# Project-MONAI/GenerativeModels

Measured on AMD Instinct MI355X. Metric: 3D volumes/sec (DDIM 50-step sample, 1x128^3), higher is better.
Workload: dtype bf16; 1 GPU; C2: 3D DiffusionModelUNet(64,128,256; 2 res blocks; mid-block attention 1 head x 256) DDIM-50 sampling of 1x1x128^3 volumes, 1 volume per GPU per step; inference_steps=50, parallelism=1 independent replicas (batch-sharded, no data-path collective), hip_graph=False, self_launched=False

## Files before the change

generativemodels_amd/csrc/small_ops.hip:

```cpp
#include <cstdlib>
#include "attn_common.h"
#include "conv_common.h"

struct LinearRowsExtra {
  const float* ln_g; const float* ln_b; float ln_eps;
  void* y1; void* y2; long long y12_ld; int split;
  const int* off_dev; long long off_mul;
  const float* kv_ws; int kv_dh;
  const float* mlp_p; int mlp_nj; const void* mlp_x1; const float* mlp_b2; void* mlp_x0;
  const float* pre_scale; const float* pre_shift; long long ss_ld; int rows_per_sample;
  void* vt; int vt_c0; int vt_dh;
  const double* gn_stats[2]; int gn_S[2]; int gn_C[2]; const float* gn_gamma; const float* gn_beta; float gn_eps; int gn_groups; int gn_N;
};

__device__ __forceinline__ float kv_merge_one(const float* __restrict__ ws, int BH, int dh, int bh, int c) {
  constexpr int NS = GM_DECODE_KV_SPLITS;
  const float* o = ws + (long long)bh * NS * dh + c;
  const float* m = ws + (long long)BH * NS * dh + (long long)bh * NS;
  const float* l = m + (long long)BH * NS;
  float ms[NS], ls[NS], os[NS];
#pragma unroll
  for (int s = 0; s < NS; ++s) { ms[s] = m[s]; ls[s] = l[s]; os[s] = o[(long long)s * dh]; }
  float M = -INFINITY;
#pragma unroll
// ... 58 lines not shown
    const float* bsrc = bias ? bias : reinterpret_cast<const float*>(w);
    const T* rsrc = res ? res + (long long)(row_ok ? row : 0) * res_ld : w;
#pragma unroll
    for (int i = 0; i < 4; ++i) {
      const int co = co0 + 4 * q + i;
      bia[i] = bsrc[bias ? (co < cout ? co : cout - 1) : 0];
      rsd[i] = ElemIO<T>::ld(rsrc + (res ? (co < cout ? co : cout - 1) : 0));
    }
  }
  f32x4_t acc = (f32x4_t){0.f, 0.f, 0.f, 0.f};
  constexpr int U = 4;
  for (int c0 = 0; c0 < nchunks; c0 += U) {
    uint4 wf[U], xf[U];
    float asc[U][VECW], ash[U][VECW];
#pragma unroll
    for (int u = 0; u < U; ++u) {
      const int c = c0 + u < nchunks ? c0 + u : nchunks - 1;
      wf[u] = *reinterpret_cast<const uint4*>(wrow + (long long)c * cout_pad * BK);
      const bool ok = row_ok & (c * BK + q * VECW + VECW <= cin);
      const uint4 v = *reinterpret_cast<const uint4*>(ok ? xrow + c * BK : x);
      xf[u] = make_uint4(ok ? v.x : 0u, ok ? v.y : 0u, ok ? v.z : 0u, ok ? v.w : 0u);
      if (ex.pre_scale) {
        const int cb = c * BK + q * VECW + VECW <= cin ? c * BK + q * VECW : 0;
        const long long off = (long long)((row_ok ? row : 0) / ex.rows_per_sample) * ex.ss_ld + cb;
#pragma unroll
        for (int i = 0; i < VECW; i += 4) {
          const float4 a = *reinterpret_cast<const float4*>(ex.pre_scale + off + i), b2 = *reinterpret_cast<const float4*>(ex.pre_shift + off + i);
          asc[u][i] = a.x; asc[u][i + 1] = a.y; asc[u][i + 2] = a.z; asc[u][i + 3] = a.w;
          ash[u][i] = b2.x; ash[u][i + 1] = b2.y; ash[u][i + 2] = b2.z; ash[u][i + 3] = b2.w;
        }
      }
    }
#pragma unroll
    for (int u = 0; u < U; ++u) {
      if (c0 + u >= nchunks) break;
      uint4 b = xf[u];
      if (pre_act || ex.ln_g || ex.pre_scale) {
        float v[VECW];
        Vec16<T>::unpack(b, v);
        if (ex.pre_scale) {
          const bool okc = row_ok & ((c0 + u) * BK + q * VECW + VECW <= cin);
#pragma unroll
          for (int i = 0; i < VECW; ++i) v[i] = okc ? v[i] * asc[u][i] + ash[u][i] : 0.f;
        }
        if (ex.ln_g) {
          const int cbase = (c0 + u) * BK + q * VECW;
          const bool ok = row_ok & (cbase + VECW <= cin);
#pragma unroll
          for (int i = 0; i < VECW; ++i) v[i] = ok ? (v[i] - mean) * rstd * ex.ln_g[cbase + i] + (ex.ln_b ? ex.ln_b[cbase + i] : 0.f) : 0.f;
        }
        if (pre_act) {
          conv_act_vec(v, pre_act, PRECISE);
        }
        b = Vec16<T>::pack(v);
      }
      Mma<T>::run(wf[u], b, acc);
    }
  }
  if (!row_ok) return;
#pragma unroll
  for (int i = 0; i < 4; ++i) {
    const int co = co0 + 4 * q + i;
    if (co < cout) {
      float v = acc[i] + (bias ? bia[i] : 0.f);
      v = conv_post_act(v, post_act);
      if (res) v += rsd[i];
      if (ex.split > 0 && co >= ex.split) {
        T* dst = reinterpret_cast<T*>(co < 2 * ex.split ? ex.y1 : ex.y2) + (ex.off_dev ? (long long)(*ex.off_dev) * ex.off_mul : 0);
        ElemIO<T>::st(dst + (long long)row * ex.y12_ld + (co - (co < 2 * ex.split ? ex.split : 2 * ex.split)), v);
      } else {
        ElemIO<T>::st(y + (long long)row * y_ld + co, v);
        if (ex.vt && co >= ex.vt_c0) {
          const int cch = co - ex.vt_c0, L = ex.rows_per_sample;
          const int smp = row / L, key = row - smp * L;
          const int pos = (key & ~31) + ((key & 15) >> 2) * 8 + ((key >> 4) & 1) * 4 + (key & 3);
          const int heads = (cout - ex.vt_c0) / ex.vt_dh;
          ElemIO<T>::st(reinterpret_cast<T*>(ex.vt) + ((long long)(smp * heads + cch / ex.vt_dh) * ex.vt_dh + cch % ex.vt_dh) * L + pos, v);
        }
      }
    }
  }
}

template <typename T, int NB, bool GN>
__global__ __launch_bounds__(256) void token_gemm_wide_kernel(const T* __restrict__ x, long long x_ld, const T* __restrict__ w, const float* __restrict__ bias,
                                                             const T* __restrict__ res, long long res_ld, T* __restrict__ y, long long y_ld, int rows, int cin,
                                                             int cout, int pre_act, int post_act, LinearRowsExtra ex) {
  constexpr int BK = ConvTraits<T>::BK, VECW = ConvTraits<T>::VECW;
  constexpr bool PRECISE = sizeof(T) == 4;
  const int lane = threadIdx.x & 63, wave = threadIdx.x >> 6;
  const int l15 = lane & 15, q = lane >> 4;
  const int cout_pad = (cout + 15) & ~15;
  const int co0 = blockIdx.x * (16 * NB);
  const int r0 = (blockIdx.y * 4 + wave) * 16;
  extern __shared__ __attribute__((aligned(16))) char gn_smem[];
  if constexpr (GN) {
    float* tab = reinterpret_cast<float*>(gn_smem);
    double* csum = reinterpret_cast<double*>(gn_smem + 2 * (size_t)cin * 4);
    const int n = (blockIdx.y * 64) / ex.rows_per_sample;
    const int cpg = cin / ex.gn_groups;
    for (int c = threadIdx.x; c < cin; c += 256) {
      const double2 v = gn_short_channel_sum(ex.gn_stats[0], ex.gn_S[0], ex.gn_C[0], ex.gn_stats[1], ex.gn_S[1], ex.gn_C[1], ex.gn_N, n, c);
      csum[2 * c] = v.x; csum[2 * c + 1] = v.y;
    }
    __syncthreads();
    for (int c = threadIdx.x; c < cin; c += 256) {
      const int g = c / cpg;
      double a = 0.0, b2 = 0.0;
      for (int j = 0; j < cpg; ++j) { a += csum[2 * (g * cpg + j)]; b2 += csum[2 * (g * cpg + j) + 1]; }
      float sc1, sh1;
      gn_short_scale_shift(a, b2, cpg, (long long)ex.rows_per_sample, ex.gn_eps, ex.gn_gamma ? ex.gn_gamma[c] : 1.f, ex.gn_beta ? ex.gn_beta[c] : 0.f, sc1, sh1);
      tab[c] = sc1;
      tab[cin + c] = sh1;
    }
    __syncthreads();
  }
  if (r0 >= rows) return;
  const int row = r0 + l15;
  const bool row_ok = row < rows;
  const int rowc = row_ok ? row : rows - 1;
  const int nchunks = cin / BK;
  const T* xrow = x + (long long)rowc * x_ld + q * VECW;
  int wblk[NB];
#pragma unroll
  for (int nb = 0; nb < NB; ++nb) wblk[nb] = co0 + 16 * nb < cout_pad ? co0 + 16 * nb : cout_pad - 16;
  const T* wrow = w + (long long)l15 * BK + q * VECW;
  const long long aoff = ex.pre_scale ? (long long)(rowc / ex.rows_per_sample) * ex.ss_ld + q * VECW : 0;
  float bia[NB][4];
  uint2 rsd[NB];
  const bool vec4 = (cout & 3) == 0 && (y_ld & 3) == 0 && (reinterpret_cast<uintptr_t>(y) & (4 * sizeof(T) - 1)) == 0 &&
                    (!res || ((res_ld & 3) == 0 && (reinterpret_cast<uintptr_t>(res) & (4 * sizeof(T) - 1)) == 0));
#pragma unroll
  for (int nb = 0; nb < NB; ++nb) {
#pragma unroll
    for (int i = 0; i < 4; ++i) {
      const int co = wblk[nb] + 4 * q + i;
      bia[nb][i] = bias ? bias[co < cout ? co : cout - 1] : 0.f;
    }
    rsd[nb] = make_uint2(0u, 0u);
    if (sizeof(T) == 2 && res && vec4) {
      const int co = wblk[nb] + 4 * q;
      rsd[nb] = *reinterpret_cast<const uint2*>(res + (long long)rowc * res_ld + (co + 3 < cout ? co : 0));
    }
  }
  f32x4_t acc[NB];
#pragma unroll
  for (int nb = 0; nb < NB; ++nb) acc[nb] = (f32x4_t){0.f, 0.f, 0.f, 0.f};
  constexpr int U = 2;
  for (int c0 = 0; c0 < nchunks; c0 += U) {
    uint4 wf[U][NB], xf[U];
    float asc[U][VECW], ash[U][VECW];
#pragma unroll
    for (int u = 0; u < U; ++u) {
      const int c = c0 + u < nchunks ? c0 + u : nchunks - 1;
      xf[u] = *reinterpret_cast<const uint4*>(xrow + c * BK);
#pragma unroll
      for (int nb = 0; nb < NB; ++nb) wf[u][nb] = *reinterpret_cast<const uint4*>(wrow + ((long long)c * cout_pad + wblk[nb]) * BK);
      if (GN) {
        const float* tab = reinterpret_cast<const float*>(gn_smem) + c * BK + q * VECW;
#pragma unroll
        for (int i = 0; i < VECW; i += 4) {
          const float4 a = *reinterpret_cast<const float4*>(tab + i), b2 = *reinterpret_cast<const float4*>(tab + cin + i);
          asc[u][i] = a.x; asc[u][i + 1] = a.y; asc[u][i + 2] = a.z; asc[u][i + 3] = a.w;
          ash[u][i] = b2.x; ash[u][i + 1] = b2.y; ash[u][i + 2] = b2.z; ash[u][i + 3] = b2.w;
        }
      } else if (ex.pre_scale) {
#pragma unroll
        for (int i = 0; i < VECW; i += 4) {
          const float4 a = *reinterpret_cast<const float4*>(ex.pre_scale + aoff + c * BK + i), b2 = *reinterpret_cast<const float4*>(ex.pre_shift + aoff + c * BK + i);
          asc[u][i] = a.x; asc[u][i + 1] = a.y; asc[u][i + 2] = a.z; asc[u][i + 3] = a.w;
          ash[u][i] = b2.x; ash[u][i + 1] = b2.y; ash[u][i + 2] = b2.z; ash[u][i + 3] = b2.w;
        }
      }
    }
#pragma unroll
    for (int u = 0; u < U; ++u) {
      if (c0 + u >= nchunks) break;
      uint4 b = row_ok ? xf[u] : make_uint4(0u, 0u, 0u, 0u);
      if (pre_act || ex.pre_scale || GN) {
        float v[VECW];
        Vec16<T>::unpack(b, v);
        if (ex.pre_scale || GN) {
#pragma unroll
          for (int i = 0; i < VECW; ++i) v[i] = row_ok ? v[i] * asc[u][i] + ash[u][i] : 0.f;
        }
        if (pre_act) conv_act_vec(v, pre_act, PRECISE);
        b = Vec16<T>::pack(v);
      }
#pragma unroll
      for (int nb = 0; nb < NB; ++nb) Mma<T>::run(wf[u][nb], b, acc[nb]);
    }
  }
  if (!row_ok) return;
#pragma unroll
  for (int nb = 0; nb < NB; ++nb) {
    if (co0 + 16 * nb >= cout_pad) break;
    const int cob = co0 + 16 * nb + 4 * q;
    float o[4];
    float rs[4] = {0.f, 0.f, 0.f, 0.f};
    if (res) {
      if (sizeof(T) == 2 && vec4) {
        rs[0] = __uint_as_float(rsd[nb].x << 16); rs[1] = __uint_as_float(rsd[nb].x & 0xffff0000u);
        rs[2] = __uint_as_float(rsd[nb].y << 16); rs[3] = __uint_as_float(rsd[nb].y & 0xffff0000u);
      } else {
#pragma unroll
        for (int i = 0; i < 4; ++i) rs[i] = cob + i < cout ? ElemIO<T>::ld(res + (long long)row * res_ld + cob + i) : 0.f;
      }
    }
#pragma unroll
    for (int i = 0; i < 4; ++i) {
      float v = acc[nb][i] + (bias ? bia[nb][i] : 0.f);
      v = conv_post_act(v, post_act);
      if (res) v += rs[i];
      o[i] = v;
    }
    if (vec4) {
      if (cob < cout) {
        if (sizeof(T) == 2) *reinterpret_cast<uint2*>(y + (long long)row * y_ld + cob) = make_uint2(pack_bf16x2(o[0], o[1]), pack_bf16x2(o[2], o[3]));
        else *reinterpret_cast<float4*>(y + (long long)row * y_ld + cob) = make_float4(o[0], o[1], o[2], o[3]);
      }
    } else {
#pragma unroll
      for (int i = 0; i < 4; ++i)
        if (cob + i < cout) ElemIO<T>::st(y + (long long)row * y_ld + cob + i, o[i]);
    }
    if (ex.vt && cob + 3 >= ex.vt_c0) {
      const int L = ex.rows_per_sample, smp = row / L, key = row - smp * L;
      const int pos = (key & ~31) + ((key & 15) >> 2) * 8 + ((key >> 4) & 1) * 4 + (key & 3);
      const int heads = (cout - ex.vt_c0) / ex.vt_dh;
#pragma unroll
      for (int i = 0; i < 4; ++i) {
        const int cch = cob + i - ex.vt_c0;
        if (cch >= 0 && cob + i < cout)
          ElemIO<T>::st(reinterpret_cast<T*>(ex.vt) + ((long long)(smp * heads + cch / ex.vt_dh) * ex.vt_dh + cch % ex.vt_dh) * L + pos, o[i]);
      }
    }
  }
}

static int gm_token_gemm_wide_rows = 2048, gm_token_gemm_wide_nb = 0;
extern "C" void gm_token_gemm_set_wide(int min_rows, int nb) {
  gm_token_gemm_wide_rows = min_rows < 0 ? 2048 : min_rows;
  gm_token_gemm_wide_nb = (nb == 2 || nb == 3 || nb == 4) ? nb : 0;
}

#define GM_ROWS_KCH 4

template <typename T, bool SRC_LDS>
__device__ __forceinline__ void stage_rows(const T* __restrict__ x, long long x_ld, T* xs, int rows, int cin, const float* __restrict__ ln_g,
                                           const float* __restrict__ ln_b, float ln_eps, int pre_act) {
  constexpr int VECW = ConvTraits<T>::VECW;
  constexpr bool PRECISE = sizeof(T) == 4;
  const int lane = threadIdx.x & 63, wave = threadIdx.x >> 6;
  const float* gsrc = ln_g ? ln_g : reinterpret_cast<const float*>(x ? (const void*)x : (const void*)xs);
  const float* bsrc = ln_b ? ln_b : gsrc;
  const float bmul = ln_b ? 1.f : 0.f;
  for (int r = wave; r < rows; r += 4) {
    float v[GM_ROWS_KCH][VECW], g[GM_ROWS_KCH][VECW], bb[GM_ROWS_KCH][VECW];
    bool ok[GM_ROWS_KCH];
#pragma unroll
    for (int k = 0; k < GM_ROWS_KCH; ++k) {
      const int ch = (k * 64 + lane) * VECW;
      ok[k] = ch + VECW <= cin;
      const int c = ok[k] ? ch : 0;
      const uint4 raw = SRC_LDS ? *reinterpret_cast<const uint4*>(xs + (long long)r * cin + c) : *reinterpret_cast<const uint4*>(x + (long long)r * x_ld + c);
      Vec16<T>::unpack(raw, v[k]);
      if (ln_g) {
#pragma unroll
        for (int i = 0; i < VECW; i += 4) {
          const float4 tg = *reinterpret_cast<const float4*>(gsrc + c + i), tb = *reinterpret_cast<const float4*>(bsrc + c + i);
          g[k][i] = tg.x; g[k][i + 1] = tg.y; g[k][i + 2] = tg.z; g[k][i + 3] = tg.w;
          bb[k][i] = tb.x; bb[k][i + 1] = tb.y; bb[k][i + 2] = tb.z; bb[k][i + 3] = tb.w;
        }
      }
    }
    if (ln_g) {
      float sum = 0.f;
#pragma unroll
      for (int k = 0; k < GM_ROWS_KCH; ++k)
#pragma unroll
        for (int i = 0; i < VECW; ++i) sum += ok[k] ? v[k][i] : 0.f;
      const float mean = wave_sum(sum) / (float)cin;
      float sq = 0.f;
#pragma unroll
      for (int k = 0; k < GM_ROWS_KCH; ++k)
#pragma unroll
        for (int i = 0; i < VECW; ++i) sq += ok[k] ? (v[k][i] - mean) * (v[k][i] - mean) : 0.f;
      const float rstd = 1.0f / sqrtf(wave_sum(sq) / (float)cin + ln_eps);
#pragma unroll
      for (int k = 0; k < GM_ROWS_KCH; ++k)
#pragma unroll
        for (int i = 0; i < VECW; ++i) v[k][i] = (v[k][i] - mean) * rstd * g[k][i] + bb[k][i] * bmul;
    }
#pragma unroll
    for (int k = 0; k < GM_ROWS_KCH; ++k) {
      if (pre_act) conv_act_vec(v[k], pre_act, PRECISE);
      if (ok[k]) *reinterpret_cast<uint4*>(xs + (long long)r * cin + (k * 64 + lane) * VECW) = Vec16<T>::pack(v[k]);
    }
  }
}

template <typename T, int STAGE, int XF>
__global__ __launch_bounds__(256) void linear_rows_ksplit_kernel(const T* __restrict__ x, long long x_ld, const T* __restrict__ w,
                                                                const float* __restrict__ bias, const T* __restrict__ res, long long res_ld,
                                                                T* __restrict__ y, long long y_ld, int rows, int cin, int cout, int pre_act,
                                                                int post_act, LinearRowsExtra ex) {
  constexpr int BK = ConvTraits<T>::BK, VECW = ConvTraits<T>::VECW;
  constexpr bool STAGED = STAGE != 0 || XF != 0;
  __shared__ float part[3][64][4];
  extern __shared__ __attribute__((aligned(16))) char staged_raw[];
  T* xs = reinterpret_cast<T*>(staged_raw);
  const int lane = threadIdx.x & 63, wave = threadIdx.x >> 6;
  const int l15 = lane & 15, q = lane >> 4;
  const int cout_pad = (cout + 15) & ~15;
  const int co0 = blockIdx.x * 16;
  const int row = l15;
  const bool row_ok = row < rows;
  const int nchunks = (cin + BK - 1) / BK;
  const T* wrow = w + ((long long)(co0 + l15)) * BK + q * VECW;
  constexpr int U = 4;
  uint4 wf[U], xf[U];
// ... 142 lines not shown
    const uint4 v = *reinterpret_cast<const uint4*>(xs + (ok ? (long long)row * C + c * BK + q * VECW : 0));
    return make_uint4(ok ? v.x : 0u, ok ? v.y : 0u, ok ? v.z : 0u, ok ? v.w : 0u);
  };
  f32x4_t acc = (f32x4_t){0.f, 0.f, 0.f, 0.f};
  for (int c0 = 0; c0 < nchunks; c0 += U) {
    if (c0 != 0) {
#pragma unroll
      for (int u = 0; u < U; ++u) wf[u] = *reinterpret_cast<const uint4*>(w1row + (long long)(c0 + u < nchunks ? c0 + u : nchunks - 1) * mpad * BK);
    }
#pragma unroll
    for (int u = 0; u < U; ++u)
      if (c0 + u < nchunks) Mma<T>::run(wf[u], xvec(c0 + u), acc);
  }
#pragma unroll
  for (int i = 0; i < 4; ++i) {
    float v = acc[i] + (b1 ? b1v[i] : 0.f);
    v = conv_post_act(v, act);
    ElemIO<T>::st(&hs[l15][wave * 16 + 4 * q + i], row_ok ? v : 0.f);
  }
  __syncthreads();
  uint4 hf[HC];
#pragma unroll
  for (int c = 0; c < HC; ++c) hf[c] = *reinterpret_cast<const uint4*>(&hs[l15][c * BK + q * VECW]);
  float* Pj = P + (long long)j * rows * C;
#pragma unroll
  for (int g = 0; g < GMAX; ++g) {
    const int grp = wave + 4 * g;
    if (grp < ngroups) {
      f32x4_t a2 = (f32x4_t){0.f, 0.f, 0.f, 0.f};
#pragma unroll
      for (int c = 0; c < HC; ++c) Mma<T>::run(w2f[g][c], hf[c], a2);
      if (row_ok) {
#pragma unroll
        for (int i = 0; i < 4; ++i) {
          const int co = grp * 16 + 4 * q + i;
          if (co < C) Pj[(long long)row * C + co] = a2[i];
        }
      }
    }
  }
}

static bool linear_rows_takes_ksplit(int rows, int cin, int dtype) {
  static const bool ksplit = !(getenv("GM_LINEAR_KSPLIT") && getenv("GM_LINEAR_KSPLIT")[0] == '0');
  const int bk = dtype == GM_F32 ? 16 : 32, vecw = dtype == GM_F32 ? 4 : 8;
  return ksplit && (cin + bk - 1) / bk >= 8 && rows <= 16 && cin <= 64 * vecw * GM_ROWS_KCH && (long long)rows * cin * (dtype == GM_F32 ? 4 : 2) <= 48 * 1024;
}

static int linear_rows_launch(const void* x, long long x_ld, const void* w, const float* bias, const void* res, long long res_ld, void* y,
                              long long y_ld, int rows, int cin, int cout, int pre_act, int post_act, int dtype, const LinearRowsExtra& ex,
                              void* stream) {
  GM_REQUIRE((x || ex.kv_ws || ex.mlp_p) && w && y, "null pointer");
  GM_REQUIRE(rows >= 0 && cin > 0 && cout > 0, "bad geometry");
  if (rows == 0) return 0;
  const int vecw = dtype == GM_F32 ? 4 : 8;
  GM_REQUIRE(cin % vecw == 0 && x_ld % vecw == 0 && (reinterpret_cast<uintptr_t>(x) & 15) == 0, "x rows must be 16-byte vectors");
  GM_REQUIRE(!(ex.kv_ws || ex.mlp_p) || linear_rows_takes_ksplit(rows, cin, dtype), "the partial-merging prologues live in the K-split kernel");
  GM_REQUIRE(ex.split == 0 || (ex.y1 && ex.y2 && cout == 3 * ex.split), "split output needs two extra destinations and cout = 3 * split");
  hipStream_t st = (hipStream_t)stream;
  const int cout_pad = (cout + 15) & ~15;
  if (linear_rows_takes_ksplit(rows, cin, dtype) && !ex.pre_scale) {
    dim3 gk(cout_pad / 16, 1);
    const int stage = ex.kv_ws ? 1 : ex.mlp_p ? 2 : 0;
    const int xf = (ex.ln_g || pre_act) ? 1 : 0;
    const size_t smem = (stage || xf) ? (size_t)rows * cin * (dtype == GM_F32 ? 4 : 2) : 0;
#define GM_KSPLIT_LAUNCH(T, STAGE, XF)                                                                                                         \
  linear_rows_ksplit_kernel<T, STAGE, XF><<<gk, 256, smem, st>>>((const T*)x, x_ld, (const T*)w, bias, (const T*)res, res_ld, (T*)y, y_ld, rows, \
                                                                 cin, cout, pre_act, post_act, ex)
#define GM_KSPLIT_DISPATCH(T)                                                         \
  do {                                                                                \
    if (stage == 0) { if (xf) GM_KSPLIT_LAUNCH(T, 0, 1); else GM_KSPLIT_LAUNCH(T, 0, 0); } \
    else if (stage == 1) { if (xf) GM_KSPLIT_LAUNCH(T, 1, 1); else GM_KSPLIT_LAUNCH(T, 1, 0); } \
    else { if (xf) GM_KSPLIT_LAUNCH(T, 2, 1); else GM_KSPLIT_LAUNCH(T, 2, 0); }       \
  } while (0)
    if (dtype == GM_F32) GM_KSPLIT_DISPATCH(float);
    else if (dtype == GM_BF16) GM_KSPLIT_DISPATCH(bf16_raw);
    else GM_FAIL(-2, "unsupported dtype");
#undef GM_KSPLIT_DISPATCH
#undef GM_KSPLIT_LAUNCH
    GM_LAUNCH_CHECK();
  }
  const int bk = dtype == GM_F32 ? 16 : 32;
  const bool gn = ex.gn_stats[0] != nullptr;
  if ((gn || (gm_token_gemm_wide_rows > 0 && rows >= gm_token_gemm_wide_rows)) && cin % bk == 0 && cout_pad >= 32 && !ex.ln_g && !ex.kv_ws && !ex.mlp_p && ex.split == 0 &&
      !ex.off_dev && (!ex.pre_scale || ex.rows_per_sample > 0) && (dtype == GM_F32 || dtype == GM_BF16)) {
    const int nb = gm_token_gemm_wide_nb ? gm_token_gemm_wide_nb : (rows >= 8192 ? 4 : 2);
    dim3 gw((cout_pad + 16 * nb - 1) / (16 * nb), (rows + 63) / 64);
    const size_t gsm = gn ? (size_t)cin * (2 * 4 + 16) : 0;
#define GM_WIDE_LAUNCH(T, NBV)                                                                                                                                    \
  do {                                                                                                                                                            \
    if (gn) token_gemm_wide_kernel<T, NBV, true><<<gw, 256, gsm, st>>>((const T*)x, x_ld, (const T*)w, bias, (const T*)res, res_ld, (T*)y, y_ld, rows, cin, cout, \
                                                                       pre_act, post_act, ex);                                                                    \
    else token_gemm_wide_kernel<T, NBV, false><<<gw, 256, 0, st>>>((const T*)x, x_ld, (const T*)w, bias, (const T*)res, res_ld, (T*)y, y_ld, rows, cin, cout,     \
                                                                   pre_act, post_act, ex);                                                                        \
  } while (0)
    if (dtype == GM_F32) { if (nb == 2) GM_WIDE_LAUNCH(float, 2); else if (nb == 3) GM_WIDE_LAUNCH(float, 3); else GM_WIDE_LAUNCH(float, 4); }
    else { if (nb == 2) GM_WIDE_LAUNCH(bf16_raw, 2); else if (nb == 3) GM_WIDE_LAUNCH(bf16_raw, 3); else GM_WIDE_LAUNCH(bf16_raw, 4); }
#undef GM_WIDE_LAUNCH
    GM_LAUNCH_CHECK();
  }
  GM_REQUIRE(!gn, "the statistics form of the token GEMM's GroupNorm needs the wide kernel's geometry (cin a multiple of the MFMA K step, cout >= 32)");
  dim3 grid((cout_pad / 16 + 3) / 4, (rows + 15) / 16);
  if (dtype == GM_F32)
    linear_rows_kernel<float><<<grid, 256, 0, st>>>((const float*)x, x_ld, (const float*)w, bias, (const float*)res, res_ld, (float*)y, y_ld,
                                                    rows, cin, cout, pre_act, post_act, ex);
  else if (dtype == GM_BF16)
    linear_rows_kernel<bf16_raw><<<grid, 256, 0, st>>>((const bf16_raw*)x, x_ld, (const bf16_raw*)w, bias, (const bf16_raw*)res, res_ld,
                                                       (bf16_raw*)y, y_ld, rows, cin, cout, pre_act, post_act, ex);
  else
    GM_FAIL(-2, "unsupported dtype");
  GM_LAUNCH_CHECK();
}

extern "C" int gm_linear_rows(const void* x, long long x_ld, const void* w, const float* bias, const void* res, long long res_ld, void* y,
                              long long y_ld, int rows, int cin, int cout, int pre_act, int post_act, int dtype, void* stream) {
  LinearRowsExtra ex = {};
  return linear_rows_launch(x, x_ld, w, bias, res, res_ld, y, y_ld, rows, cin, cout, pre_act, post_act, dtype, ex, stream);
}

extern "C" int gm_linear_rows_affine(const void* x, long long x_ld, const float* pre_scale, const float* pre_shift, long long ss_ld, int rows_per_sample,
                                     const void* w, const float* bias, const void* res, long long res_ld, void* y, long long y_ld, int rows, int cin,
                                     int cout, int pre_act, int post_act, int dtype, void* stream) {
  GM_REQUIRE((pre_scale == nullptr) == (pre_shift == nullptr), "scale and shift come together");
  GM_REQUIRE(!pre_scale || (rows_per_sample > 0 && ss_ld % 4 == 0 && (reinterpret_cast<uintptr_t>(pre_scale) & 15) == 0 &&
                            (reinterpret_cast<uintptr_t>(pre_shift) & 15) == 0), "the affine tables are 16-byte aligned fp32 rows");
  LinearRowsExtra ex = {};
  ex.pre_scale = pre_scale; ex.pre_shift = pre_shift; ex.ss_ld = ss_ld; ex.rows_per_sample = rows_per_sample;
  return linear_rows_launch(x, x_ld, w, bias, res, res_ld, y, y_ld, rows, cin, cout, pre_act, post_act, dtype, ex, stream);
}

extern "C" int gm_linear_rows_affine_vt(const void* x, long long x_ld, const float* pre_scale, const float* pre_shift, long long ss_ld, int rows_per_sample,
                                        const void* w, const float* bias, void* y, long long y_ld, int rows, int cin, int cout, int pre_act, void* vt,
                                        int vt_c0, int vt_dh, int dtype, void* stream) {
  GM_REQUIRE((pre_scale == nullptr) == (pre_shift == nullptr), "scale and shift come together");
  GM_REQUIRE(!pre_scale || (ss_ld % 4 == 0 && (reinterpret_cast<uintptr_t>(pre_scale) & 15) == 0 && (reinterpret_cast<uintptr_t>(pre_shift) & 15) == 0),
             "the affine tables are 16-byte aligned fp32 rows");
  GM_REQUIRE(vt && dtype == GM_BF16 && rows_per_sample > 0 && rows_per_sample % 64 == 0 && rows % rows_per_sample == 0, "the V^T image needs bf16 and whole 64-key blocks per sample");
  GM_REQUIRE(vt_dh > 0 && vt_c0 >= 0 && vt_c0 < cout && (cout - vt_c0) % vt_dh == 0, "the V columns are whole heads");
  LinearRowsExtra ex = {};
  ex.pre_scale = pre_scale; ex.pre_shift = pre_shift; ex.ss_ld = ss_ld; ex.rows_per_sample = rows_per_sample;
  ex.vt = vt; ex.vt_c0 = vt_c0; ex.vt_dh = vt_dh;
  return linear_rows_launch(x, x_ld, w, bias, nullptr, 0, y, y_ld, rows, cin, cout, pre_act, 0, dtype, ex, stream);
}

extern "C" int gm_linear_rows_gn(const void* x, long long x_ld, const GmGnTables* gn, int n_samples, int rows_per_sample, const void* w, const float* bias,
                                 const void* res, long long res_ld, void* y, long long y_ld, int rows, int cin, int cout, int pre_act, int post_act, void* vt,
                                 int vt_c0, int vt_dh, int dtype, void* stream) {
  GM_REQUIRE(gn && gn->stats[0] && gn->groups > 0 && cin % gn->groups == 0 && cin <= 384, "GroupNorm tables: whole groups, at most 384 channels");
  GM_REQUIRE(gn->S[0] >= 1 && gn->S[0] <= GN_SHORT_MAX_ROWS && gn->C[0] > 0 &&
             ((gn->stats[1] == nullptr && gn->C[0] == cin) || (gn->stats[1] != nullptr && gn->S[1] >= 1 && gn->S[1] <= GN_SHORT_MAX_ROWS && gn->C[1] > 0 && gn->C[0] + gn->C[1] == cin)),
             "short statistic tables covering the input channels");
  GM_REQUIRE((reinterpret_cast<uintptr_t>(gn->stats[0]) & 15) == 0 && (reinterpret_cast<uintptr_t>(gn->stats[1]) & 15) == 0, "16-byte aligned tables");
  GM_REQUIRE(n_samples > 0 && rows_per_sample > 0 && rows_per_sample % 64 == 0 && rows == n_samples * rows_per_sample, "whole 64-row groups per sample");
  GM_REQUIRE(!vt || (dtype == GM_BF16 && vt_dh > 0 && vt_c0 >= 0 && vt_c0 < cout && (cout - vt_c0) % vt_dh == 0 && !res && post_act == 0), "the V^T image: bf16, whole heads, no residual");
  LinearRowsExtra ex = {};
  ex.rows_per_sample = rows_per_sample;
  ex.gn_stats[0] = gn->stats[0]; ex.gn_stats[1] = gn->stats[1]; ex.gn_S[0] = gn->S[0]; ex.gn_S[1] = gn->stats[1] ? gn->S[1] : 0;
  ex.gn_C[0] = gn->C[0]; ex.gn_C[1] = gn->stats[1] ? gn->C[1] : 0;
  ex.gn_gamma = gn->gamma; ex.gn_beta = gn->beta; ex.gn_eps = gn->eps; ex.gn_groups = gn->groups; ex.gn_N = n_samples;
  ex.vt = vt; ex.vt_c0 = vt_c0; ex.vt_dh = vt_dh;
  return linear_rows_launch(x, x_ld, w, bias, res, res_ld, y, y_ld, rows, cin, cout, pre_act, post_act, dtype, ex, stream);
}

extern "C" int gm_linear_rows_ln(const void* x, long long x_ld, const float* ln_g, const float* ln_b, float ln_eps, const void* w,
                                 const float* bias, void* y, long long y_ld, void* y1, void* y2, long long y12_ld, int split, int rows, int cin,
                                 int cout, int post_act, int dtype, const int* off_dev, long long off_mul, void* stream) {
// ... 526 lines not shown
```

generativemodels_amd/ops.py:

```python
from __future__ import annotations

import contextlib
import ctypes as C
import math
import os
import threading
import weakref
from typing import Optional, Sequence

import torch

from . import _native as nat
from ._native import GmAttnBwdDesc, GmAttnDesc, GmConvDesc, GmGnTables, GmKlParams, GmStepParams, GmWgradDesc, check, lib

_DT = {torch.float32: 0, torch.bfloat16: 1}
ACT = {"none": 0, "silu": 1, "relu": 2}
ACT_BWD = {"none": 0, "silu": 1, "relu": 2, "leakyrelu": 3}
POST_ACT = {"none": 0, "relu": 1, "tanh": 2, "sigmoid": 3, "silu": 4, "swish": 4, "leakyrelu": 5, "gelu": 6}


def dt_code(dtype: torch.dtype) -> int:
    try:
        return _DT[dtype]
    except KeyError:
# ... 605 lines not shown
    if GN_APPLY_POLICY == "prologue":
        return True
    if GN_APPLY_POLICY == "pass":
        return False
    if x.dtype != torch.bfloat16 or x.shape[-1] % 8 != 0:
        return True
    if x.numel() >= (1 << 22):
        return False
    vox = x.numel() // max(x.shape[0] * x.shape[-1], 1)
    return not (x.dim() == 5 and x.shape[-1] % 32 == 0 and vox <= 4096)


def layernorm(x: torch.Tensor, gamma: Optional[torch.Tensor], beta: Optional[torch.Tensor], eps: float = 1e-5) -> torch.Tensor:
    require_device(x)
    out = torch.empty(x.shape, dtype=x.dtype, device=x.device)
    check(lib().gm_layernorm(x.data_ptr(), arena_ld(x), out.data_ptr(), arena_ld(out), _ptr(as_f32(gamma)), _ptr(as_f32(beta)),
                             rows_of(x), x.shape[-1], float(eps), dt_code(x.dtype), _stream()), "gm_layernorm")
    return out


def geglu(x: torch.Tensor) -> torch.Tensor:
    require_device(x)
    inner = x.shape[-1] // 2
    out = torch.empty((*x.shape[:-1], inner), dtype=x.dtype, device=x.device)
    check(lib().gm_geglu(x.data_ptr(), arena_ld(x), out.data_ptr(), arena_ld(out), rows_of(x), inner, dt_code(x.dtype), _stream()),
          "gm_geglu")
    return out


def _clog2(v: int) -> int:
    return max(0, (int(v) - 1).bit_length())


def _tile_bits(total_bits: int, out_dims):
    caps = [_clog2(d) for d in out_dims]
    bits = [0, 0, 0]
    for _ in range(total_bits):
        cand = [i for i in (2, 1, 0) if bits[i] < caps[i]]
        if not cand:
            bits[2] += 1
            continue
        i = min(cand, key=lambda j: bits[j])
        bits[i] += 1
    return bits


def _tile_bits_fast(total_bits: int, out_dims):
    caps = [_clog2(d) for d in out_dims]
    bits = [0, 0, min(4, caps[2], total_bits)]
    for _ in range(total_bits - bits[2]):
        cand = [i for i in (1, 0) if bits[i] < caps[i]]
        if not cand:
            bits[2] += 1
            continue
        i = min(cand, key=lambda j: bits[j])
        bits[i] += 1
    return bits


_CFG_TILES = {}


def _cfg_tile(cfg: int):
    if cfg not in _CFG_TILES:
        bm, bn = C.c_int(), C.c_int()
        check(lib().gm_conv_cfg_tile(cfg, C.byref(bm), C.byref(bn)), "gm_conv_cfg_tile")
        _CFG_TILES[cfg] = (bm.value, bn.value)
    return _CFG_TILES[cfg]


COUT1_MARCH_LTD = os.environ.get("GM_CONV_COUT1_LTD")
COUT1_MARCH_LTW_128B = int(os.environ.get("GM_CONV_COUT1_LTW", "4"))


_CONV_DEBUG_FLAGS = 0
_SK_STAMPS = None
_CONV_TIMELINE_BUFFER = None

SMALL_LINEAR_ROWS = 64
TOKEN_GEMM = os.environ.get("GM_TOKEN_GEMM", "1") != "0"
TOKEN_GEMM_MAX_ROWS = int(os.environ.get("GM_TOKEN_GEMM_MAX_ROWS", "32768"))
TOKEN_GEMM_MAX_CIN = 512
TOKEN_GEMM_MAX_FLOP = float(os.environ.get("GM_TOKEN_GEMM_MAX_FLOP", "2.0e9"))
DMA_CONV = True
DMA_CONV_MIN_VOXELS = 1 << 8
LDS_SOFT_LIMIT = 80 * 1024
LDS_HARD_LIMIT = 160 * 1024


def _choose_conv_cfg(desc: GmConvDesc, n_vox_out: int, force_cfg: Optional[int] = None, only: Optional[tuple] = None, exclude: tuple = ()):
    cout = desc.Cout
    if force_cfg is not None:
        order = [force_cfg]
    elif cout <= 16:
        order = [3, 4, 2]
    elif cout <= 64:
        order = [10, 8, 5, 0, 4, 2] if n_vox_out * desc.N >= (1 << 20) else [8, 5, 0, 4, 2]
    else:
        order = [10, 9, 6, 1, 4, 2] if n_vox_out * desc.N >= (1 << 20) else [9, 6, 1, 4, 2]
    if force_cfg is None and n_vox_out * desc.N >= DMA_CONV_MIN_VOXELS:
        if cout == 1:
            order = ([20, 13] if COUT1_MARCH else [13]) + order
        if desc.Cin <= 4:
            order = [12] + order
    if force_cfg is None and cout > 16 and DMA_CONV and n_vox_out * desc.N >= DMA_CONV_MIN_VOXELS:
        tiles = desc.N * -(-desc.Do // 4) * -(-desc.Ho // 4) * -(-desc.Wo // 16) * -(-cout // 64)
        wide = (bool(desc.pre_scale is None or not desc.pre_scale) or DMA_WIDE_WAVES_PRE) and tiles >= DMA_WIDE_WAVE_MIN_TILES and DMA_WIDE_WAVES
        order = ([15] if desc.sd == 2 else ([14, 11] if wide else [11])) + order
    if (force_cfg is None and NARROW_N_2D and DMA_CONV and desc.kd == 1 and desc.Ds == 1 and desc.kh == 3 and desc.kw == 3
            and ((desc.sh == 1 and desc.sw == 1) or (NARROW_N_2D_STRIDE2 and desc.sh == 2 and desc.sw == 2))
            and 2.0 * n_vox_out * desc.N * cout * desc.Cin * 9 * desc.sh * desc.sw <= NARROW_N_2D_MAX_FLOP):
        order = [25] + order
    if force_cfg is None and n_vox_out * desc.N <= 256 * 64:
        dma_first = [c for c in order if c in (11, 12, 15, 18, 19)]
        rest = [c for c in order if c not in (11, 12, 15, 18, 19)]
        order = dma_first + [c for c in rest if _cfg_tile(c)[0] <= 64] + [c for c in rest if _cfg_tile(c)[0] > 64]
    order = [c for c in order if (only is None or c in only) and c not in exclude]
    best = None
    for cfg in order:
        bm, _ = _cfg_tile(cfg)
        tb = _tile_bits_fast if cfg >= 5 else _tile_bits
        bits = tb(bm.bit_length() - 1, (desc.Do, desc.Ho, desc.Wo))
        if cfg == 20:
            ltw = (COUT1_MARCH_LTW_128B if desc.Cin * (4 if desc.dtype == 0 else 2) == 128 else 4)
            cols = desc.N * -(-desc.Ho // 8) * -(-desc.Wo // (1 << ltw))
            want = 512 if (ltw == 4 and desc.Cin * (4 if desc.dtype == 0 else 2) == 128) else 256
            ltd = 5
            while ltd > 2 and cols * -(-desc.Do // (1 << ltd)) < want:
                ltd -= 1
            if COUT1_MARCH_LTD is not None:
                ltd = int(COUT1_MARCH_LTD)
            bits = [ltd, 3, ltw]
        if cfg in (11, 12, 14, 15, 16, 18, 19, 24, 25):
            bits = {11: [2, 2, 4], 12: [2, 2, 4], 14: [2, 2, 4], 15: [1, 2, 4], 16: [3, 2, 4], 18: [3, 2, 4], 19: [3, 2, 4], 24: [2, 2, 4], 25: [0, 4, 4]}[cfg]
        desc.cfg, desc.ltd, desc.lth, desc.ltw = cfg, bits[0], bits[1], bits[2]
        lds = lib().gm_conv_lds_bytes(C.byref(desc))
        soft = LDS_HARD_LIMIT if cfg >= 5 else LDS_SOFT_LIMIT
        if 0 < lds <= soft:
            return
        if 0 < lds <= LDS_HARD_LIMIT and best is None:
            best = (cfg, bits)
    if best is None:
        raise ValueError("convolution geometry needs more than 160 KiB of LDS per tile (kernel/stride/dilation too large)")
    desc.cfg, (desc.ltd, desc.lth, desc.ltw) = best[0], best[1]


def _attach_conv_stats(d: GmConvDesc, out: torch.Tensor, n: int, cout: int) -> None:
    slots = lib().gm_conv_stats_slots(C.byref(d))
    if slots > 0:
        cst = torch.empty((slots, n, cout, 2), dtype=torch.float64, device=out.device)
        d.stats = cst.data_ptr()
        out._gm_cstats = cst


def _conv_subpixel(x, weight, bias, rowvec, res, post_act, out, want_stats, n, cin, cout, src, packed=None, label="mode3 (executed flops: 8 of the 27 taps)"):
    dtype = x.dtype
    out_sp = tuple(2 * v for v in src)
    out_shape = (n, *out_sp, cout)
    if out is None:
        out = torch.empty(out_shape, dtype=dtype, device=x.device)
    elif tuple(out.shape) != out_shape or out.dtype != dtype:
        raise ValueError(f"out has shape {tuple(out.shape)}, expected {out_shape}")
    d = GmConvDesc()
    if packed is None:
        packed = packed_subpixel_weight(weight, dtype)
    d.in_mode, d.fd, d.fh, d.fw = 3, 2, 2, 2
# ... 73 lines not shown
        x, x2 = x.parts
    require_device(x, x2, weight, bias, rowvec, res, out)
    nsp = x.dim() - 2
    if nsp < 1 or nsp > 3:
        raise ValueError("conv expects (N, *spatial, C) with 1-3 spatial axes")

    def two_pass():
        parts = [x] if x2 is None else [x, x2]
        if pre is None and x2 is None:
            raise AssertionError
        xa = torch.empty((*x.shape[:-1], sum(t.shape[-1] for t in parts)), dtype=x.dtype, device=x.device)
        off = 0
        for t in parts:
            c_t = t.shape[-1]
            if pre is not None:
                gn_apply(t, pre[0][:, off:off + c_t], pre[1][:, off:off + c_t], pre_act, out=xa[..., off:off + c_t])
            else:
                copy_channels(t, xa[..., off:off + c_t])
            off += c_t
        return conv(xa, weight, bias, kernel=kernel, stride=stride, padding=padding, dilation=dilation, pad_hi=pad_hi, upsample=upsample,
                    transposed=transposed, output_padding=output_padding, rowvec=rowvec, res=res, post_act=post_act, out=out, packed=packed,
                    cout=cout, force_cfg=force_cfg, want_stats=want_stats, skip=skip, allow_subpixel=allow_subpixel, ksplit=ksplit, vt=vt)

    def tup(v):
        v = tuple(v) if isinstance(v, (tuple, list)) else (int(v),) * nsp
        if len(v) != nsp:
            raise ValueError("per-axis argument has the wrong length")
        return v

    def pad3(v, fill):
        return (fill,) * (3 - nsp) + tuple(v)

    k = pad3(tup(kernel), 1)
    s = pad3(tup(stride), 1)
    plo = pad3(tup(padding), 0)
    phi = pad3(tup(pad_hi if pad_hi is not None else padding), 0)
    dil = pad3(tup(dilation), 1)
    opad = pad3(tup(output_padding), 0)
    n, cin = x.shape[0], x.shape[-1] + (0 if x2 is None else x2.shape[-1])
    src = pad3(tuple(x.shape[1:-1]), 1)
    dtype = x.dtype
    if x2 is not None and (x2.shape[:-1] != x.shape[:-1] or x2.dtype != dtype):
        raise ValueError("the two parts of a concatenated input must agree outside the channel dim")
    if packed is None:
        cout = weight.shape[1] if transposed else weight.shape[0]
        wcin = weight.shape[0] if transposed else weight.shape[1]
        if wcin != cin:
            raise ValueError(f"input has {cin} channels but the weight expects {wcin}")

    def panel():
        return packed if packed is not None else packed_conv_weight(weight, dtype, transposed)
    rows = n * math.prod(src)
    vecw = 16 // x.element_size()
    if (rows <= SMALL_LINEAR_ROWS and x2 is None and k == (1, 1, 1) and s == (1, 1, 1) and not transposed and not upsample and pre is None
            and rowvec is None and not want_stats and skip is None and force_cfg is None and cin % vecw == 0
            and arena_ld(x) % vecw == 0 and x.data_ptr() % 16 == 0 and plo == (0, 0, 0) and phi == (0, 0, 0)):
        out_shape = (*x.shape[:-1], cout)
        if out is None:
            out = torch.empty(out_shape, dtype=dtype, device=x.device)
        elif tuple(out.shape) != out_shape or out.dtype != dtype:
            raise ValueError(f"out has shape {tuple(out.shape)}, expected {out_shape}")
        if res is not None and (tuple(res.shape) != out_shape or res.dtype != dtype):
            raise ValueError(f"residual has shape {tuple(res.shape)} / {res.dtype}, expected {out_shape} / {dtype}")
        b32 = as_f32(bias) if bias is not None else None
        _timed(f"linear_rows<{str(dtype).split('.')[-1]}>", dict(flops=2.0 * rows * cin * cout, bytes=float(x.element_size() * cin * cout), shape=f"{rows}x{cin}->{cout}"),
               lambda: check(lib().gm_linear_rows(x.data_ptr(), arena_ld(x), panel().data_ptr(), _ptr(b32), _ptr(res), 0 if res is None else arena_ld(res),
                                                  out.data_ptr(), arena_ld(out), rows, cin, cout, ACT[pre_act], POST_ACT[post_act], dt_code(dtype),
                                                  _stream()), "gm_linear_rows"))
        return out
    if (EDGE_2D_AS_3D and nsp == 2 and x2 is None and packed is None and weight is not None and weight.dim() == 4 and not transposed and not upsample
            and cin <= 4 and k == (1, 3, 3) and s == (1, 1, 1) and dil == (1, 1, 1) and plo == (0, 1, 1) and phi == (0, 1, 1) and pre is None
            and pre_act == "none" and skip is None and force_cfg is None and ksplit is None and cout % vecw == 0 and rows >= DMA_CONV_MIN_VOXELS):
        def embed():
            w5 = torch.zeros((weight.shape[0], weight.shape[1], 3, 3, 3), dtype=weight.dtype, device=weight.device)
            w5[:, :, 1] = weight.detach()
            return w5
        got = conv(x.unsqueeze(1), _cached(weight, ("centre_plane_3d",), embed), bias, kernel=3, padding=1, rowvec=rowvec,
                   res=None if res is None else res.unsqueeze(1), post_act=post_act, out=None if out is None else out.unsqueeze(1), want_stats=want_stats)
        y = out if out is not None else got.squeeze(1)
        st = getattr(got, "_gm_cstats", None)
        if st is not None:
            y._gm_cstats = st
        return y
    if (TOKEN_GEMM and SMALL_LINEAR_ROWS < rows <= TOKEN_GEMM_MAX_ROWS and cin <= TOKEN_GEMM_MAX_CIN and 2.0 * rows * cin * cout <= TOKEN_GEMM_MAX_FLOP
            and x2 is None and k == (1, 1, 1) and s == (1, 1, 1) and not upsample and rowvec is None and not want_stats and skip is None
            and force_cfg is None and ksplit is None and cin % vecw == 0 and arena_ld(x) % vecw == 0 and x.data_ptr() % 16 == 0
            and plo == (0, 0, 0) and phi == (0, 0, 0) and opad == (0, 0, 0)):
        out_shape = (*x.shape[:-1], cout)
        if out is None:
            out = torch.empty(out_shape, dtype=dtype, device=x.device)
        elif tuple(out.shape) != out_shape or out.dtype != dtype:
            raise ValueError(f"out has shape {tuple(out.shape)}, expected {out_shape}")
        if res is not None and (tuple(res.shape) != out_shape or res.dtype != dtype):
            raise ValueError(f"residual has shape {tuple(res.shape)} / {res.dtype}, expected {out_shape} / {dtype}")
        b32 = as_f32(bias) if bias is not None else None
        if GN_IN_TOKEN_GEMM and isinstance(pre, GnRecipe) and pre._done is None and not transposed:
            l_tok = rows // n
            want_vt = (vt is not None and res is None and post_act == "none" and dtype == torch.bfloat16 and l_tok % 64 == 0)
            if (pre.n == n and sum(pre.cs) == cin and cin <= 384 and cin % (64 // x.element_size()) == 0 and cout >= 32 and l_tok % 64 == 0
                    and cin % pre.groups == 0 and all(st.shape[0] <= GN_IN_CONSUMER_MAX_ROWS for st in pre.stats) and (vt is None or want_vt)):
                g = GmGnTables()
                for i, st in enumerate(pre.stats):
                    g.stats[i], g.S[i], g.C[i] = st.data_ptr(), st.shape[0], pre.cs[i]
                g.gamma, g.beta, g.eps, g.groups = _ptr(pre.gamma), _ptr(pre.beta), pre.eps, pre.groups
                vws, vt_c0, vt_dh = vt if want_vt else (None, 0, 0)
                _timed(f"token_gemm<{str(dtype).split('.')[-1]}>", dict(flops=2.0 * rows * cin * cout, bytes=float(x.element_size() * (rows * (cin + cout) + cin * cout)),
                                                                      shape=f"{rows}x{cin}->{cout} (GroupNorm from statistics{' +V^T image' if want_vt else ''})"),
                       lambda: check(lib().gm_linear_rows_gn(x.data_ptr(), arena_ld(x), C.byref(g), n, l_tok, panel().data_ptr(), _ptr(b32), _ptr(res),
                                                             0 if res is None else arena_ld(res), out.data_ptr(), arena_ld(out), rows, cin, cout, ACT[pre_act],
                                                             POST_ACT[post_act], None if vws is None else vws.data_ptr(), int(vt_c0), int(vt_dh), dt_code(dtype),
                                                             _stream()), "gm_linear_rows_gn"))
                if want_vt:
                    out._gm_vt_packed = True
                return out
        sc = sh = None
        if pre is not None:
            sc, sh = pre
            if sc.dtype != torch.float32 or sh.dtype != torch.float32 or sc.shape != (n, cin) or sh.shape != (n, cin) or sc.stride(-1) != 1 or sh.stride(-1) != 1 \
                    or sc.stride(0) != sh.stride(0):
                raise ValueError("pre = (scale, shift): fp32 [N, Cin] tables with a common row pitch")
        if (vt is not None and res is None and post_act == "none" and dtype == torch.bfloat16 and (rows // n) % 64 == 0
                and (sc is None or (sc.stride(0) % 4 == 0 and sc.data_ptr() % 16 == 0 and sh.data_ptr() % 16 == 0))):
            vws, vt_c0, vt_dh = vt
            _timed(f"token_gemm<{str(dtype).split('.')[-1]}>", dict(flops=2.0 * rows * cin * cout, bytes=float(x.element_size() * (rows * (cin + cout) + cin * cout)),
                                                                  shape=f"{rows}x{cin}->{cout} (+V^T image)"),
                   lambda: check(lib().gm_linear_rows_affine_vt(x.data_ptr(), arena_ld(x), _ptr(sc), _ptr(sh), 0 if sc is None else sc.stride(0), rows // n,
                                                                panel().data_ptr(), _ptr(b32), out.data_ptr(), arena_ld(out), rows, cin, cout, ACT[pre_act],
                                                                vws.data_ptr(), int(vt_c0), int(vt_dh), dt_code(dtype), _stream()), "gm_linear_rows_affine_vt"))
            out._gm_vt_packed = True
            return out
        if sc is None or (sc.stride(0) % 4 == 0 and sc.data_ptr() % 16 == 0 and sh.data_ptr() % 16 == 0):
            _timed(f"token_gemm<{str(dtype).split('.')[-1]}>", dict(flops=2.0 * rows * cin * cout, bytes=float(x.element_size() * (rows * (cin + cout) + cin * cout)),
                                                                  shape=f"{rows}x{cin}->{cout}"),
                   lambda: check(lib().gm_linear_rows_affine(x.data_ptr(), arena_ld(x), _ptr(sc), _ptr(sh), 0 if sc is None else sc.stride(0), rows // n,
                                                             panel().data_ptr(), _ptr(b32), _ptr(res), 0 if res is None else arena_ld(res), out.data_ptr(),
                                                             arena_ld(out), rows, cin, cout, ACT[pre_act], POST_ACT[post_act], dt_code(dtype), _stream()),
                                 "gm_linear_rows_affine"))
            return out
    if (upsample and x2 is None and SUBPIXEL_UPSAMPLE and allow_subpixel and nsp == 3 and k == (3, 3, 3) and s == (1, 1, 1) and plo == (1, 1, 1) and phi == (1, 1, 1)
            and dil == (1, 1, 1) and pre is None and pre_act == "none" and skip is None and force_cfg is None and weight is not None
            and cin % (64 // x.element_size()) == 0 and cout % vecw == 0 and arena_ld(x) % vecw == 0 and x.data_ptr() % 16 == 0
            and math.prod(src) * n >= DMA_CONV_MIN_VOXELS):
        got = _conv_subpixel(x, weight, bias, rowvec, res, post_act, out, want_stats, n, cin, cout, src)
        if got is not None:
            return got
    if (transposed and TRANSPOSED_S2_SUBPIXEL and x2 is None and nsp == 3 and s == (2, 2, 2) and k in ((3, 3, 3), (4, 4, 4)) and dil == (1, 1, 1)
            and plo[0] == plo[1] == plo[2] and stride2_subpixel_covers(k[0], plo[0]) and pre is None and pre_act == "none" and skip is None and force_cfg is None
            and weight is not None and all((src[i] - 1) * 2 - plo[i] - phi[i] + k[i] + opad[i] == 2 * src[i] for i in range(3))
            and cin % (64 // x.element_size()) == 0 and cout % vecw == 0 and arena_ld(x) % vecw == 0 and x.data_ptr() % 16 == 0
            and math.prod(src) * n >= DMA_CONV_MIN_VOXELS):
        got = _conv_subpixel(x, weight, bias, rowvec, res, post_act, out, want_stats, n, cin, cout, src,
                             packed=packed_stride2_dgrad_weight(weight, dtype, plo[0]),
                             label=f"transposed k{k[0]} s2 as 8 sub-pixel 2x2x2 convolutions")
        if got is not None:
            return got
    d = GmConvDesc()
    d.in_mode, d.fd, d.fh, d.fw = 0, 1, 1, 1
    act_axes = (0,) * (3 - nsp) + (1,) * nsp
    if transposed:
        if upsample:
            raise ValueError("upsample and transposed are exclusive")
        d.in_mode = 2
        d.fd, d.fh, d.fw = s
        if s == (1, 1, 1):
            d.in_mode = 0
        out_sp = tuple((src[i] - 1) * s[i] - plo[i] - phi[i] + dil[i] * (k[i] - 1) + opad[i] + 1 for i in range(3))
        conv_pad = tuple(dil[i] * (k[i] - 1) - plo[i] for i in range(3))
        conv_stride = (1, 1, 1)
    else:
        virt = src
        if upsample:
            d.in_mode = 1
            d.fd, d.fh, d.fw = tuple(2 if a else 1 for a in act_axes)
            virt = tuple(src[i] * (2 if act_axes[i] else 1) for i in range(3))
        out_sp = tuple((virt[i] + plo[i] + phi[i] - dil[i] * (k[i] - 1) - 1) // s[i] + 1 for i in range(3))
        conv_pad, conv_stride = plo, s
    if min(out_sp) <= 0:
        raise ValueError(f"convolution output would be empty: {out_sp}")
    out_shape = (n, *out_sp[3 - nsp:], cout)
# ... 969 lines not shown
```

Baseline: 1.442 volumes/s.

## Add register-resident row GEMM kernel for long-sequence QKV projection with V^T packing

Adds a token GEMM kernel that keeps each 16-row tile's full 256-wide input in registers and loops over all output channel blocks. It writes the V^T packed image for attention in the same pass, and factors the store epilogue into a shared helper. On the Python side, long-sequence bf16 QKV projections that used to exceed the token-GEMM FLOP cap are now routed to this path. GroupNorm-in-GEMM fusion is disabled for them, which can add a separate normalization pass, and weights are re-read from cache by every wave instead of being shared through LDS.

```diff
diff --git a/generativemodels_amd/csrc/small_ops.hip b/generativemodels_amd/csrc/small_ops.hip
--- a/generativemodels_amd/csrc/small_ops.hip
+++ b/generativemodels_amd/csrc/small_ops.hip
@@ -164,6 +164,40 @@
   }
 }
 
+template <typename T>
+__device__ __forceinline__ void token_gemm_store(const f32x4_t& acc, const float* bia, const float* rs, int row, int cob, T* __restrict__ y, long long y_ld,
+                                                 int cout, int post_act, bool vec4, const LinearRowsExtra& ex) {
+  float o[4];
+#pragma unroll
+  for (int i = 0; i < 4; ++i) {
+    float v = acc[i] + bia[i];
+    v = conv_post_act(v, post_act);
+    if (rs) v += rs[i];
+    o[i] = v;
+  }
+  if (vec4) {
+    if (cob < cout) {
+      if (sizeof(T) == 2) *reinterpret_cast<uint2*>(y + (long long)row * y_ld + cob) = make_uint2(pack_bf16x2(o[0], o[1]), pack_bf16x2(o[2], o[3]));
+      else *reinterpret_cast<float4*>(y + (long long)row * y_ld + cob) = make_float4(o[0], o[1], o[2], o[3]);
+    }
+  } else {
+#pragma unroll
+    for (int i = 0; i < 4; ++i)
+      if (cob + i < cout) ElemIO<T>::st(y + (long long)row * y_ld + cob + i, o[i]);
+  }
+  if (ex.vt && cob + 3 >= ex.vt_c0) {
+    const int L = ex.rows_per_sample, smp = row / L, key = row - smp * L;
+    const int pos = (key & ~31) + ((key & 15) >> 2) * 8 + ((key >> 4) & 1) * 4 + (key & 3);
+    const int heads = (cout - ex.vt_c0) / ex.vt_dh;
+#pragma unroll
+    for (int i = 0; i < 4; ++i) {
+      const int cch = cob + i - ex.vt_c0;
+      if (cch >= 0 && cob + i < cout)
+        ElemIO<T>::st(reinterpret_cast<T*>(ex.vt) + ((long long)(smp * heads + cch / ex.vt_dh) * ex.vt_dh + cch % ex.vt_dh) * L + pos, o[i]);
+    }
+  }
+}
+
 template <typename T, int NB, bool GN>
 __global__ __launch_bounds__(256) void token_gemm_wide_kernel(const T* __restrict__ x, long long x_ld, const T* __restrict__ w, const float* __restrict__ bias,
                                                              const T* __restrict__ res, long long res_ld, T* __restrict__ y, long long y_ld, int rows, int cin,
@@ -278,7 +312,6 @@
   for (int nb = 0; nb < NB; ++nb) {
     if (co0 + 16 * nb >= cout_pad) break;
     const int cob = co0 + 16 * nb + 4 * q;
-    float o[4];
     float rs[4] = {0.f, 0.f, 0.f, 0.f};
     if (res) {
       if (sizeof(T) == 2 && vec4) {
@@ -289,36 +322,85 @@
         for (int i = 0; i < 4; ++i) rs[i] = cob + i < cout ? ElemIO<T>::ld(res + (long long)row * res_ld + cob + i) : 0.f;
       }
     }
-#pragma unroll
-    for (int i = 0; i < 4; ++i) {
-      float v = acc[nb][i] + (bias ? bia[nb][i] : 0.f);
-      v = conv_post_act(v, post_act);
-      if (res) v += rs[i];
-      o[i] = v;
-    }
-    if (vec4) {
-      if (cob < cout) {
-        if (sizeof(T) == 2) *reinterpret_cast<uint2*>(y + (long long)row * y_ld + cob) = make_uint2(pack_bf16x2(o[0], o[1]), pack_bf16x2(o[2], o[3]));
-        else *reinterpret_cast<float4*>(y + (long long)row * y_ld + cob) = make_float4(o[0], o[1], o[2], o[3]);
-      }
-    } else {
-#pragma unroll
-      for (int i = 0; i < 4; ++i)
-        if (cob + i < cout) ElemIO<T>::st(y + (long long)row * y_ld + cob + i, o[i]);
-    }
-    if (ex.vt && cob + 3 >= ex.vt_c0) {
-      const int L = ex.rows_per_sample, smp = row / L, key = row - smp * L;
-      const int pos = (key & ~31) + ((key & 15) >> 2) * 8 + ((key >> 4) & 1) * 4 + (key & 3);
-      const int heads = (cout - ex.vt_c0) / ex.vt_dh;
+    token_gemm_store(acc[nb], bia[nb], res ? rs : nullptr, row, cob, y, y_ld, cout, post_act, vec4, ex);
+  }
+}
+
+template <typename T, int KC, int NB>
+__global__ __launch_bounds__(256) void token_gemm_rows_kernel(const T* __restrict__ x, long long x_ld, const T* __restrict__ w, const float* __restrict__ bias,
+                                                             T* __restrict__ y, long long y_ld, int rows, int cout, int pre_act, int post_act, LinearRowsExtra ex) {
+  constexpr int BK = ConvTraits<T>::BK, VECW = ConvTraits<T>::VECW;
+  constexpr bool PRECISE = sizeof(T) == 4;
+  const int lane = threadIdx.x & 63, wave = threadIdx.x >> 6;
+  const int l15 = lane & 15, q = lane >> 4;
+  const int cout_pad = (cout + 15) & ~15;
+  const int r0 = (blockIdx.x * 4 + wave) * 16;
+  if (r0 >= rows) return;
+  const int row = r0 + l15;
+  const bool row_ok = row < rows;
+  const int rowc = row_ok ? row : rows - 1;
+  const T* xrow = x + (long long)rowc * x_ld + q * VECW;
+  uint4 xb[KC];
+#pragma unroll
+  for (int c = 0; c < KC; ++c) xb[c] = *reinterpret_cast<const uint4*>(xrow + c * BK);
+  const long long aoff = ex.pre_scale ? (long long)(rowc / ex.rows_per_sample) * ex.ss_ld + q * VECW : 0;
+#pragma unroll
+  for (int c = 0; c < KC; ++c) {
+    uint4 b = row_ok ? xb[c] : make_uint4(0u, 0u, 0u, 0u);
+    if (pre_act || ex.pre_scale) {
+      float v[VECW];
+      Vec16<T>::unpack(b, v);
+      if (ex.pre_scale) {
+        float asc[VECW], ash[VECW];
+#pragma unroll
+        for (int i = 0; i < VECW; i += 4) {
+          const float4 a = *reinterpret_cast<const float4*>(ex.pre_scale + aoff + c * BK + i), b2 = *reinterpret_cast<const float4*>(ex.pre_shift + aoff + c * BK + i);
+          asc[i] = a.x; asc[i + 1] = a.y; asc[i + 2] = a.z; asc[i + 3] = a.w;
+          ash[i] = b2.x; ash[i + 1] = b2.y; ash[i + 2] = b2.z; ash[i + 3] = b2.w;
+        }
+#pragma unroll
+        for (int i = 0; i < VECW; ++i) v[i] = row_ok ? v[i] * asc[i] + ash[i] : 0.f;
+      }
+      if (pre_act) conv_act_vec(v, pre_act, PRECISE);
+      b = Vec16<T>::pack(v);
+    }
+    xb[c] = b;
+  }
+  const T* wrow = w + (long long)l15 * BK + q * VECW;
+  const bool vec4 = (cout & 3) == 0 && (y_ld & 3) == 0 && (reinterpret_cast<uintptr_t>(y) & (4 * sizeof(T) - 1)) == 0;
+  for (int co0 = 0; co0 < cout_pad; co0 += 16 * NB) {
+    int wblk[NB];
+#pragma unroll
+    for (int nb = 0; nb < NB; ++nb) wblk[nb] = co0 + 16 * nb < cout_pad ? co0 + 16 * nb : cout_pad - 16;
+    float bia[NB][4];
+#pragma unroll
+    for (int nb = 0; nb < NB; ++nb)
 #pragma unroll
       for (int i = 0; i < 4; ++i) {
-        const int cch = cob + i - ex.vt_c0;
-        if (cch >= 0 && cob + i < cout)
-          ElemIO<T>::st(reinterpret_cast<T*>(ex.vt) + ((long long)(smp * heads + cch / ex.vt_dh) * ex.vt_dh + cch % ex.vt_dh) * L + pos, o[i]);
-      }
-    }
-  }
-}
+        const int co = wblk[nb] + 4 * q + i;
+        bia[nb][i] = bias ? bias[co < cout ? co : cout - 1] : 0.f;
+      }
+    f32x4_t acc[NB];
+#pragma unroll
+    for (int nb = 0; nb < NB; ++nb) acc[nb] = (f32x4_t){0.f, 0.f, 0.f, 0.f};
+#pragma unroll
+    for (int c = 0; c < KC; ++c) {
+      uint4 wf[NB];
+#pragma unroll
+      for (int nb = 0; nb < NB; ++nb) wf[nb] = *reinterpret_cast<const uint4*>(wrow + ((long long)c * cout_pad + wblk[nb]) * BK);
+#pragma unroll
+      for (int nb = 0; nb < NB; ++nb) Mma<T>::run(wf[nb], xb[c], acc[nb]);
+    }
+    if (!row_ok) continue;
+#pragma unroll
+    for (int nb = 0; nb < NB; ++nb) {
+      if (co0 + 16 * nb >= cout_pad) break;
+      token_gemm_store(acc[nb], bia[nb], nullptr, row, co0 + 16 * nb + 4 * q, y, y_ld, cout, post_act, vec4, ex);
+    }
+  }
+}
+
+#define GM_TOKEN_GEMM_ROWS_MIN 16384
 
 static int gm_token_gemm_wide_rows = 2048, gm_token_gemm_wide_nb = 0;
 extern "C" void gm_token_gemm_set_wide(int min_rows, int nb) {
@@ -627,6 +709,11 @@
   }
   const int bk = dtype == GM_F32 ? 16 : 32;
   const bool gn = ex.gn_stats[0] != nullptr;
+  if (ex.vt && !gn && dtype == GM_BF16 && cin == 8 * bk && rows >= GM_TOKEN_GEMM_ROWS_MIN && cout_pad >= 64 && !res) {
+    token_gemm_rows_kernel<bf16_raw, 8, 4><<<(rows + 63) / 64, 256, 0, st>>>((const bf16_raw*)x, x_ld, (const bf16_raw*)w, bias, (bf16_raw*)y, y_ld, rows, cout,
+                                                                            pre_act, post_act, ex);
+    GM_LAUNCH_CHECK();
+  }
   if ((gn || (gm_token_gemm_wide_rows > 0 && rows >= gm_token_gemm_wide_rows)) && cin % bk == 0 && cout_pad >= 32 && !ex.ln_g && !ex.kv_ws && !ex.mlp_p && ex.split == 0 &&
       !ex.off_dev && (!ex.pre_scale || ex.rows_per_sample > 0) && (dtype == GM_F32 || dtype == GM_BF16)) {
     const int nb = gm_token_gemm_wide_nb ? gm_token_gemm_wide_nb : (rows >= 8192 ? 4 : 2);
diff --git a/generativemodels_amd/ops.py b/generativemodels_amd/ops.py
--- a/generativemodels_amd/ops.py
+++ b/generativemodels_amd/ops.py
@@ -711,6 +711,7 @@
 TOKEN_GEMM_MAX_ROWS = int(os.environ.get("GM_TOKEN_GEMM_MAX_ROWS", "32768"))
 TOKEN_GEMM_MAX_CIN = 512
 TOKEN_GEMM_MAX_FLOP = float(os.environ.get("GM_TOKEN_GEMM_MAX_FLOP", "2.0e9"))
+QKV_ROWS_MIN = 16384
 DMA_CONV = True
 DMA_CONV_MIN_VOXELS = 1 << 8
 LDS_SOFT_LIMIT = 80 * 1024
@@ -950,7 +951,8 @@
         if st is not None:
             y._gm_cstats = st
         return y
-    if (TOKEN_GEMM and SMALL_LINEAR_ROWS < rows <= TOKEN_GEMM_MAX_ROWS and cin <= TOKEN_GEMM_MAX_CIN and 2.0 * rows * cin * cout <= TOKEN_GEMM_MAX_FLOP
+    qkv_long = vt is not None and rows >= QKV_ROWS_MIN and cin == 256 and dtype == torch.bfloat16 and res is None and post_act == "none"
+    if (TOKEN_GEMM and SMALL_LINEAR_ROWS < rows <= TOKEN_GEMM_MAX_ROWS and cin <= TOKEN_GEMM_MAX_CIN and (2.0 * rows * cin * cout <= TOKEN_GEMM_MAX_FLOP or qkv_long)
             and x2 is None and k == (1, 1, 1) and s == (1, 1, 1) and not upsample and rowvec is None and not want_stats and skip is None
             and force_cfg is None and ksplit is None and cin % vecw == 0 and arena_ld(x) % vecw == 0 and x.data_ptr() % 16 == 0
             and plo == (0, 0, 0) and phi == (0, 0, 0) and opad == (0, 0, 0)):
@@ -962,7 +964,7 @@
         if res is not None and (tuple(res.shape) != out_shape or res.dtype != dtype):
             raise ValueError(f"residual has shape {tuple(res.shape)} / {res.dtype}, expected {out_shape} / {dtype}")
         b32 = as_f32(bias) if bias is not None else None
-        if GN_IN_TOKEN_GEMM and isinstance(pre, GnRecipe) and pre._done is None and not transposed:
+        if GN_IN_TOKEN_GEMM and isinstance(pre, GnRecipe) and pre._done is None and not transposed and not qkv_long:
             l_tok = rows // n
             want_vt = (vt is not None and res is None and post_act == "none" and dtype == torch.bfloat16 and l_tok % 64 == 0)
             if (pre.n == n and sum(pre.cs) == cin and cin <= 384 and cin % (64 // x.element_size()) == 0 and cout >= 32 and l_tok % 64 == 0
```

After: 1.439 volumes/s (median of 2 runs). Within noise of the previous version (-0.3%).
